# nabeelscicom/DistilCodec_nabeel

Hardware: AMD Instinct MI355X
Metric: 24 kHz samples/s encode+decode at 1/8 GPU; code-index bit-exact vs CPU (higher is better)
Workload: dtype f32

## Files before the change

### distilcodec_nabeel_amd/csrc/dcx_api.cpp

```cpp
#include "dcx_host.h"

namespace {

void prof_collect(dcx_codec* h) {
  if (h->pending.empty()) return;
  hipDeviceSynchronize();
  for (auto& r : h->pending) {
    float ms = 0.f;
    hipEventElapsedTime(&ms, h->events[r.ev0], h->events[r.ev1]);
    h->prof_launches[r.id] += 1;
    h->prof_ms[r.id] += ms;
    h->prof_flops[r.id] += r.flops;
    h->prof_bytes[r.id] += r.bytes;
  }
  h->pending.clear();
  h->ev_used = 0;
}

constexpr int kPlanMagic = 0x52414731, kPlanHead = 8;
enum { PLAN_MAGIC = 0, PLAN_BATCH, PLAN_FRAMES, PLAN_SAMPLES, PLAN_T16, PLAN_T4, PLAN_RUN, PLAN_RW };
constexpr int64_t kRaggedMaxSamples = INT32_MAX, kRaggedMaxFrames = 1 << 20, kRaggedMaxBatch = 1 << 20;
int64_t plan_words(int64_t batch) { return kPlanHead + 5 * (batch + 1); }

bool seg_from_plan(const int32_t* host, const int32_t* dev, int64_t batch, int64_t samples, int64_t frames,
// ... 473 lines not shown
  if (cin % 16 || cout % 32) return DCX_ERR_INVALID_ARG;
  if (transposed && (k % stride || (k - stride) % 2 || stride > dcx::kMaxPhases)) return DCX_ERR_INVALID_ARG;
  if (!transposed && (k % 2 == 0)) return DCX_ERR_INVALID_ARG;
  auto c = new (std::nothrow) dcx_conv();
  if (!c) return DCX_ERR_OOM;
  dcx_codec* h = &c->scratch;
  HostTensor wt;
  const int64_t n = (int64_t)cin * cout * k;
  wt.shape = transposed ? std::vector<int64_t>{cin, cout, k} : std::vector<int64_t>{cout, cin, k};
  wt.data.assign(weight, weight + n);
  h->host["c.weight"] = wt;
  HostTensor bt;
  bt.shape = {cout};
  if (bias) bt.data.assign(bias, bias + cout); else bt.data.assign(cout, 0.f);
  h->host["c.bias"] = bt;
  const int code = build_conv(h, cin, cout, k, dilation, transposed != 0, stride, c->w);
  h->host.clear();
  if (code != DCX_OK) {
    dcx_conv_destroy(c);
    return code;
  }
  *out = c;
  return DCX_OK;
}

int dcx_conv_forward(dcx_conv* c, int32_t gemm_mode, const float* x, int32_t batch, int64_t lin, float* y,
                     float* y_silu, const float* res, int32_t epi, void* stream) {
  if (!c || !x || batch <= 0 || lin <= 0 || (!y && !y_silu)) return DCX_ERR_INVALID_ARG;
  if (epi != dcx::EPI_BIAS && epi != dcx::EPI_GELU && epi != dcx::EPI_RES) return DCX_ERR_INVALID_ARG;
  if (epi == dcx::EPI_RES && !res) return DCX_ERR_INVALID_ARG;
  dcx_codec* h = &c->scratch;
  h->gemm_mode = gemm_mode;
  hipStream_t s = (hipStream_t)stream;
  CAct xa(x, nullptr);
  if (gemm_mode != DCX_GEMM_F32 && gemm_mode != DCX_GEMM_X6 && gemm_mode != DCX_GEMM_BF16) return DCX_ERR_INVALID_ARG;
  if (gemm_mode != DCX_GEMM_F32 && !f32_input_ok(c->w)) {
    const size_t need = (size_t)batch * lin * c->w.cin * 3;
    if (!grow(c->planes, c->planes_cap, need)) return DCX_ERR_OOM;
    const bool h3 = c->h3 && (c->w.taps >= 2 ? takes_h3_conv(h, c->w, lin) : takes_h3(h, c->w));
    if (h3) {
      const long long rows = (long long)batch * lin;
      const size_t words = (size_t)batch + (size_t)std::max<long long>(batch, rows);
      if (!grow(c->range, c->range_cap, words)) return DCX_ERR_OOM;
      float* am = reinterpret_cast<float*>(c->range);
      int* ash = c->range + batch;
      xa.r = Rng{};
      if (c->w.taps >= 2) {
        if (dcx::launch_h2_ranged(x, nullptr, c->planes, batch, lin, c->w.cin, 0, 0.f, am, ash, h->rflag, s) != hipSuccess)
          return fail(h, DCX_ERR_HIP, "h3 input split (per clip) failed");
        xa.r.ash = ash;
        xa.r.amax = am;
      } else {
        if (dcx::launch_h2_rows(x, c->planes, rows, c->w.cin, ash, s) != hipSuccess)
          return fail(h, DCX_ERR_HIP, "h3 input split (per row) failed: Cin must be 256, 512, 768 or 1024");
        xa.r.ash_row = ash;
      }
      xa.h2 = true;
    } else if (dcx::launch_split_planes(x, c->planes, (long long)batch * lin, c->w.cin, 0, s) != hipSuccess) {
      return DCX_ERR_HIP;
    }
    xa.p = c->planes;
  }
  ConvCall cc = framed(xa, batch, (int)lin, c->w.cin);
  cc.y = y;
  cc.y2 = y_silu;
  cc.res = res;
  cc.epi = epi;
  return run_conv(h, c->w, cc, s);
}

void dcx_conv_destroy(dcx_conv* c) {
  if (!c) return;
  if (c->planes) hipFree(c->planes);
  if (c->range) hipFree(c->range);
  for (void* p : c->scratch.allocs) hipFree(p);
  delete c;
}

const char* dcx_conv_last_kernel(const dcx_conv* c) { return c ? c->scratch.last_kname : ""; }

int dcx_conv_set_knob(dcx_conv* c, const char* name, int32_t value) {
  if (!c || !name) return DCX_ERR_INVALID_ARG;
  const auto k = knob_slot(name);
  if (!k) return fail(&c->scratch, DCX_ERR_INVALID_ARG, std::string("unknown knob: ") + name);
  c->scratch.knobs.*k = value;
  return DCX_OK;
}

int dcx_conv_set_h3(dcx_conv* c, int32_t on) {
  if (!c) return DCX_ERR_INVALID_ARG;
  c->h3 = on != 0;
  return DCX_OK;
}

int dcx_profile_enable(dcx_codec* h, int32_t on) {
  if (!h) return DCX_ERR_INVALID_ARG;
  h->prof = on != 0;
  return DCX_OK;
}

int dcx_profile_reset(dcx_codec* h) {
  if (!h) return DCX_ERR_INVALID_ARG;
  prof_collect(h);
  for (size_t i = 0; i < h->prof_names.size(); ++i) {
    h->prof_launches[i] = 0;
    h->prof_ms[i] = h->prof_flops[i] = h->prof_bytes[i] = 0;
  }
// ... 33 lines not shown
```

### distilcodec_nabeel_amd/csrc/dcx_conv_h3.hip

```cpp
#include "dcx_conv_common.h"
#include "dcx_conv_launch.h"
#include "dcx_conv_pingpong.h"

namespace dcx {

DCX_DIAG_FILE(h3)

typedef _Float16 f16x8 __attribute__((ext_vector_type(8)));

template <int BM, int BN>
__device__ __forceinline__ bool ragged_tile_done(const ConvParams& p, const ConvParams& pr, int wg, int b, int ph) {
  int q0, co0;
  tile_origin<BM, BN>(p, wg, q0, co0);
  if (!tile_dead(p, pr, b, q0)) return false;
  epilogue_dead<BM, BN, 512>(p, pr, q0, co0, b, ph);
  return true;
}

template <int BN, int HALO, bool RAG = false>
__device__ __forceinline__ void x3dq_tile(const ConvParams& p, const ConvParams& pr, const int wg, const int b, const int ph) {
  constexpr int BM = 32768 / BN, WN = BN / 64, WM = 8 / WN;
  constexpr int NA = HALO ? 2 : 3;
  constexpr int WR = BM / WM, WC = BN / WN, TM = WR / 16, TN = WC / 16;
  constexpr int AR = BM + HALO;
  constexpr int A_G = AR / 16, B_G = BN / 16;
  constexpr int A_PW = A_G / 4, B_PW = B_G / 4;
  constexpr int ABUF = AR * 128, BBUF = BN * 128;
  constexpr int LDS_B = NA * ABUF + 3 * BBUF;
  static_assert(WR == 64 && WC == 64 && A_G % 4 == 0 && B_G % 4 == 0 && AR % 64 == 0, "tile shape");
  static_assert(LDS_B <= 160 * 1024, "LDS");
  __shared__ __attribute__((aligned(16))) unsigned short lds[LDS_B / 2];

  if constexpr (RAG)
    if (ragged_tile_done<BM, BN>(p, pr, wg, b, ph)) return;
  const TileGeo g = tile_geo<BM, BN, WN>(p, wg, ph, p.Cin / 32);
  const int lane = g.lane, group = g.group, gw = g.gw, wm = g.wm, wn = g.wn, q0 = g.q0, co0 = g.co0;
  const int nchunks = g.nchunks, taps = g.taps, nsteps = g.nsteps, lo_rel = g.lo_rel, row0 = g.row0;
  const int arow = p.ldx * 4;
  const __amdgpu_buffer_rsrc_t rx = x_desc<4, HALO>(p, b, row0, BM);
  const int rbase = HALO ? row0 : 0;
  const __amdgpu_buffer_rsrc_t rw = __builtin_amdgcn_make_buffer_rsrc(
      (void*)(p.w3 + (long long)ph * taps * nchunks * p.Cout * 64), 0, taps * nchunks * p.Cout * 128, 0x00020000);

  int a_off[A_PW], b_off[B_PW];
#pragma unroll
  for (int i = 0; i < A_PW; ++i) {
    const int u = (group * A_G + i * 4 + gw) * 64;
    const int pc = u / AR, row = u - pc * AR + lane;
    a_off[i] = (rbase + row) * arow + (pc & 3) * 32 + (pc >> 2) * 16;
  }
#pragma unroll
  for (int i = 0; i < B_PW; ++i) {
    const int u = (group * B_G + i * 4 + gw) * 64;
    const int pc = u / BN, col = u - pc * BN + lane;
    b_off[i] = (co0 + col) * 128 + (pc & 3) * 32 + (pc >> 2) * 16;
  }
  unsigned short* const a_dst = lds + (group * A_G + gw) * 512;
  unsigned short* const b_dst = lds + NA * ABUF / 2 + (group * B_G + gw) * 512;
  [[maybe_unused]] bool in_loop = false;
  auto dma_step = [&](int c, int m, int slot) {
#ifdef DCX_X3_NODMA
    if (in_loop) return 0;
#endif
    int n = B_PW;
    if (m == 0) {
#pragma unroll
      for (int i = 0; i < A_PW; ++i)
        dma16(rx, a_dst + (HALO ? (c & 1) : slot) * (ABUF / 2) + i * 2048, a_off[i] + c * 128, 0);
      n += A_PW;
    }
    const int soff = (m * nchunks + c) * p.Cout * 128;
#pragma unroll
    for (int i = 0; i < B_PW; ++i) dma16(rw, b_dst + slot * (BBUF / 2) + i * 2048, b_off[i], soff);
    return n;
  };

  const int l15 = lane & 15, kg = lane >> 4;
  const int pah = kg * AR * 16, pal = (4 + kg) * AR * 16;
  const int pbh = kg * BN * 16, pbl = (4 + kg) * BN * 16;
  const char* const ldsb = reinterpret_cast<const char*>(lds);
  const int bcol = NA * ABUF + (wn * WC + l15) * 16;
  s16x8 aq[TM][2], bq[TN][2];
  auto readF = [&](int c, int m, int slot) {
    const char* a = ldsb + (HALO ? (c & 1) : slot) * ABUF + (wm * WR + m * p.in_step - lo_rel + l15) * 16;
    const char* bb = ldsb + bcol + slot * BBUF;
#pragma unroll
    for (int j = 0; j < TN; ++j) {
      bq[j][0] = *reinterpret_cast<const s16x8*>(bb + j * 256 + pbh);
      bq[j][1] = *reinterpret_cast<const s16x8*>(bb + j * 256 + pbl);
    }
#pragma unroll
    for (int i = 0; i < TM; ++i) {
      aq[i][0] = *reinterpret_cast<const s16x8*>(a + i * 256 + pah);
      aq[i][1] = *reinterpret_cast<const s16x8*>(a + i * 256 + pal);
    }
  };
  f32x4 acc[TM][TN];
  zero_acc(acc);
  auto mfma = [&]() {
    __builtin_amdgcn_s_setprio(1);
#pragma unroll
    for (int k = 0; k < 3; ++k) {
      const int sa = k == 1 ? 1 : 0, sb = k == 0 ? 1 : 0;
#pragma unroll
      for (int i = 0; i < TM; ++i)
#pragma unroll
        for (int j = 0; j < TN; ++j)
          acc[i][j] = __builtin_amdgcn_mfma_f32_16x16x32_f16(__builtin_bit_cast(f16x8, aq[i][sa]),
                                                             __builtin_bit_cast(f16x8, bq[j][sb]), acc[i][j], 0, 0, 0);
    }
    __builtin_amdgcn_s_setprio(0);
  };

  const StepPos l3 = pingpong3_prologue(nsteps, taps, dma_step);
  const EpiPre epre = epi_range_pre<HALO == 0 ? 3 : 0>(p, pr, b);
  const float unscale = __builtin_bit_cast(float, __builtin_amdgcn_readfirstlane(__builtin_bit_cast(int,
      __builtin_ldexpf(1.0f, -(p.w3_shift + (pr.x_ash ? pr.x_ash[b] : pr.x_ash_c))))));
  pingpong3_drain();
  in_loop = true;
  pingpong3_loop<true>(group, nsteps, taps, l3, dma_step, readF, mfma);
#pragma unroll
  for (int i = 0; i < TM; ++i)
#pragma unroll
    for (int j = 0; j < TN; ++j) acc[i][j] *= unscale;
// ... 1 lines not shown
}

template <int BN, int HALO, bool RAG = false>
__global__ void __launch_bounds__(512, 2) conv_gemm_x3dq(const ConvParams p) {
  int wg, b, ph;
  flat_tile(((p.Lq + 32768 / BN - 1) / (32768 / BN)) * (p.Cout / BN), p.batch, wg, b, ph);
  x3dq_tile<BN, HALO, RAG>(p, p, wg, b, ph);
}

template <int BN, bool RAG = false>
__global__ void __launch_bounds__(512, 2) conv_gemm_x3dq_group(const ConvGroup g) {
  ConvParams p;
  int local, b;
  const ConvParams& pr = group_member(g, p, local, b);
  x3dq_tile<BN, 64, RAG>(p, pr, local, b, 0);
}

template <int HALO, bool SPLIT, int BN = 256, bool RAG = false>
__device__ __forceinline__ void x3dw_tile(const ConvParams& p, const ConvParams& pr, const int wg, const int b, const int ph) {
  constexpr int BM = BN == 256 ? 256 : 384, WN = BN / 128, WM = 8 / WN;
  constexpr int WR = BM / WM, WC = 128, TM = WR / 16, TN = WC / 16;
  constexpr int AR = BM + HALO;
  constexpr int A_N = AR / 8, B_N = BN / 8;
  constexpr int A_PW = A_N / 4;
  constexpr int ABUF = AR * 128, BBUF = BN * 128;
  constexpr int NA = 2;
  constexpr int LDS_B = NA * ABUF + 2 * BBUF;
  static_assert(A_N % 4 == 0 && B_N % 4 == 0 && AR % 64 == 0, "tile shape");
  static_assert(LDS_B + 16 <= 160 * 1024, "LDS");
  __shared__ __attribute__((aligned(16))) unsigned short lds[LDS_B / 2 + 8];
  unsigned int* const rd_cnt = reinterpret_cast<unsigned int*>(lds + LDS_B / 2);

  const int tid = threadIdx.x, lane = tid & 63;
  [[maybe_unused]] const int wave = tid >> 6;
  const int group = __builtin_amdgcn_readfirstlane(tid >> 8);
  const int gw = __builtin_amdgcn_readfirstlane((tid >> 6) & 3);
  const int wm = wave / WN, wn = wave % WN;
  const int ntiles = p.Cout / BN;
  const int mt = wg / ntiles, nt = wg - mt * ntiles;
  const int q0 = mt * BM, co0 = nt * BN;
  if (RAG && tile_dead(p, pr, b, q0)) {
    epilogue_dead<BM, BN, 512>(p, pr, q0, co0, b, ph);
    return;
  }
  const int nchunks = p.Cin / 32;
  const int taps = p.taps;
  const int nsteps = nchunks * taps;
  const int lo_rel = p.in_step < 0 ? (taps - 1) * p.in_step : 0;
  const int row0 = q0 + p.in_base[ph] + lo_rel;
  const int arow = p.ldx * 4;
  const __amdgpu_buffer_rsrc_t rx = x_desc<4, HALO>(p, b, row0, BM);
  const int rbase = HALO ? row0 : 0;
  const __amdgpu_buffer_rsrc_t rw = __builtin_amdgcn_make_buffer_rsrc(
      (void*)(p.w3 + (long long)ph * taps * nchunks * p.Cout * 64), 0, taps * nchunks * p.Cout * 128, 0x00020000);

  const int a_lane = (rbase + lane) * arow;
  const int b_lane = (co0 + lane) * 128;
  [[maybe_unused]] bool in_loop = false;
  auto dmaA1 = [&](int c, int slot, int i) {
#ifdef DCX_X3_NODMA
    if (in_loop) return;
#endif
    const int k = i * 4 + gw;
    const int u = k * 64, pc = u / AR, row = u - pc * AR;
    const int abuf = HALO ? (c & 1) : slot;
    dma16(rx, lds + abuf * (ABUF / 2) + k * 512, a_lane + row * arow + (pc & 3) * 32 + (pc >> 2) * 16 + c * 128, 0);
  };
#ifndef DCX_X3W_BG0_DIV
#define DCX_X3W_BG0_DIV 2
#endif
  constexpr int B_G0 = !SPLIT ? B_N : HALO ? B_N / DCX_X3W_BG0_DIV : 0;
  constexpr int B_W0 = B_G0 / 4, B_W1 = (B_N - B_G0) / 4;
  auto dmaB1 = [&](int c, int m, int slot, int i) {
#ifdef DCX_X3_NODMA
    if (in_loop) return;
#endif
    const int k = (group ? B_G0 : 0) + i * 4 + gw;
    const int u = k * 64, pc = u / BN, col = u - pc * BN;
    dma16(rw, lds + NA * ABUF / 2 + slot * (BBUF / 2) + k * 512, b_lane + col * 128 + (pc & 3) * 32 + (pc >> 2) * 16,
          (m * nchunks + c) * p.Cout * 128);
  };
  auto dma_step = [&](int c, int m, int slot) {
    if (m == 0) {
#pragma unroll
      for (int i = 0; i < A_PW; ++i) dmaA1(c, slot, i);
    }
#pragma unroll
    for (int i = 0; i < B_W0; ++i) dmaB1(c, m, slot, i);
  };
  auto dma_step1 = [&](int c, int m, int slot) {
#pragma unroll
    for (int i = 0; i < B_W1; ++i) dmaB1(c, m, slot, i);
  };

  const int l15 = lane & 15, kg = lane >> 4;
  const char* const ldsb = reinterpret_cast<const char*>(lds);
  const char* const a_rd = ldsb + kg * AR * 16 + (wm * WR + l15) * 16;
  const char* const b_rd = ldsb + NA * ABUF + kg * BN * 16 + (wn * WC + l15) * 16;
  s16x8 aq[TM][2], bq[TN][2];
  auto readF = [&](int c, int m, int slot) {
    const char* a = a_rd + ((HALO ? (c & 1) : slot) * ABUF + (m * p.in_step - lo_rel) * 16);
    const char* bb = b_rd + slot * BBUF;
#pragma unroll
    for (int j = 0; j < TN; ++j) {
      bq[j][0] = *reinterpret_cast<const s16x8*>(bb + j * 256);
      bq[j][1] = *reinterpret_cast<const s16x8*>(bb + j * 256 + 4 * BN * 16);
    }
#pragma unroll
    for (int i = 0; i < TM; ++i) {
      aq[i][0] = *reinterpret_cast<const s16x8*>(a + i * 256);
      aq[i][1] = *reinterpret_cast<const s16x8*>(a + i * 256 + 4 * AR * 16);
    }
  };
  f32x4 acc[TM][TN];
  zero_acc(acc);
  auto mfma = [&]() {
    __builtin_amdgcn_s_setprio(1);
#pragma unroll
    for (int k = 0; k < 3; ++k) {
      const int sa = k == 1 ? 1 : 0, sb = k == 0 ? 1 : 0;
#pragma unroll
      for (int i = 0; i < TM; ++i) {
#pragma unroll
        for (int j = 0; j < TN; ++j)
          acc[i][j] = __builtin_amdgcn_mfma_f32_16x16x32_f16(__builtin_bit_cast(f16x8, aq[i][sa]),
                                                             __builtin_bit_cast(f16x8, bq[j][sb]), acc[i][j], 0, 0, 0);
      }
    }
    __builtin_amdgcn_s_setprio(0);
  };

  int cl = 0, ml = 0;
  if (SPLIT && tid == 0) *rd_cnt = 0u;
// ... 213 lines not shown
```

### distilcodec_nabeel_amd/csrc/dcx_misc.hip

```cpp
#include "dcx_kernels.h"
#include "dcx_planes.h"
#include "dcx_ln.h"

#include <algorithm>

namespace dcx {

template <int NV>
__global__ void __launch_bounds__(256) ln_rows_kernel(const float* __restrict__ x, float* __restrict__ y,
                                                       unsigned short* __restrict__ y6, int y6c, const float* __restrict__ w,
                                                       const float* __restrict__ b, long long rows, float eps, int cf,
                                                       int* ash_row, float* amax_row) {
  const int lane = threadIdx.x & 63;
  const long long row = (long long)blockIdx.x * 4 + (threadIdx.x >> 6);
  if (row >= rows) return;
  constexpr int C = 256 * NV;
  f32x4 v[NV];
#pragma unroll
  for (int i = 0; i < NV; ++i) v[i] = *reinterpret_cast<const f32x4*>(x + row * C + (lane + 64 * i) * 4);
  ln_finish<NV>(v, C, eps, cf, w, b, y ? y + row * C : nullptr, y6, y6c, row, lane, ash_row, amax_row);
}

hipError_t launch_ln_rows(const float* x, float* y, unsigned short* y6, int y6c, const float* w, const float* b,
                          long long rows, int C, float eps, int cf, hipStream_t s, int* ash_row, float* amax_row) {
// ... 288 lines not shown
    m = fmaxf(m, fmaxf(fmaxf(fabsf(v.x), fabsf(v.y)), fmaxf(fabsf(v.z), fabsf(v.w))));
  }
  range_report(m, amax, b, __builtin_inff(), nullptr, range_cur(amax, b));
}

__global__ void __launch_bounds__(256) h2_ranged_kernel(const float* __restrict__ x, float* __restrict__ yf,
                                                         unsigned short* __restrict__ y6, long long L, int C, int silu,
                                                         float floor, const float* __restrict__ amax, int* ash,
                                                         int* rflag, const int* __restrict__ clip_len, int len_mul) {
  const int b = blockIdx.y;
  const long long live4 = clip_len ? std::min<long long>(L, (long long)max(clip_len[b], 0) * len_mul) * C / 4 : L * C / 4;
  const float bound = fmaxf(amax[b], floor);
  const int sh = h2_shift(bound);
  const float sc = __builtin_ldexpf(1.0f, sh);
  if (blockIdx.x == 0 && threadIdx.x == 0) {
    ash[b] = sh;
    if (rflag && !(bound <= 3.0e38f)) atomicOr(rflag, RANGE_NONFINITE);
  }
  const long long n4 = L * C / 4, base = (long long)b * L * C;
  for (long long i4 = (long long)blockIdx.x * 256 + threadIdx.x; i4 < n4; i4 += (long long)gridDim.x * 256) {
    const long long i = base + i4 * 4;
    const f32x4 v = i4 < live4 ? *reinterpret_cast<const f32x4*>(x + i) : f32x4{0.f, 0.f, 0.f, 0.f};
    float o[4];
#pragma unroll
    for (int e = 0; e < 4; ++e) o[e] = silu ? v[e] * __builtin_amdgcn_rcpf(1.0f + __expf(-v[e])) : v[e];
    if (yf) *reinterpret_cast<f32x4*>(yf + i) = f32x4{o[0], o[1], o[2], o[3]};
    store_h2_4(y6, i / C, C, (int)(i % C), o[0], o[1], o[2], o[3], sc);
  }
}

template <int NV>
__global__ void __launch_bounds__(256) h2_rows_kernel(const float* __restrict__ x, unsigned short* __restrict__ y6,
                                                       long long rows, int* __restrict__ ash_row) {
  const int lane = threadIdx.x & 63;
  const long long row = (long long)blockIdx.x * 4 + (threadIdx.x >> 6);
  if (row >= rows) return;
  constexpr int C = 256 * NV;
  f32x4 v[NV];
  float am = 0.f;
#pragma unroll
  for (int i = 0; i < NV; ++i) {
    v[i] = *reinterpret_cast<const f32x4*>(x + row * C + (lane + 64 * i) * 4);
    am = fmaxf(am, fmaxf(fmaxf(fabsf(v[i].x), fabsf(v[i].y)), fmaxf(fabsf(v[i].z), fabsf(v[i].w))));
  }
#pragma unroll
  for (int off = 32; off >= 1; off >>= 1) am = fmaxf(am, __shfl_xor(am, off, 64));
  const int sh = h2_shift(am);
  const float sc = __builtin_ldexpf(1.0f, sh);
  if (lane == 0) ash_row[row] = sh;
#pragma unroll
  for (int i = 0; i < NV; ++i) store_h2_4(y6, row, C, (lane + 64 * i) * 4, v[i].x, v[i].y, v[i].z, v[i].w, sc);
}

hipError_t launch_h2_rows(const float* x, unsigned short* y6, long long rows, int C, int* ash_row, hipStream_t s) {
  if (!x || !y6 || !ash_row || rows < 0) return hipErrorInvalidValue;
  if (rows == 0) return hipSuccess;
  dim3 grid((unsigned)((rows + 3) / 4)), block(256);
  switch (C) {
    case 256: hipLaunchKernelGGL(h2_rows_kernel<1>, grid, block, 0, s, x, y6, rows, ash_row); break;
    case 512: hipLaunchKernelGGL(h2_rows_kernel<2>, grid, block, 0, s, x, y6, rows, ash_row); break;
    case 768: hipLaunchKernelGGL(h2_rows_kernel<3>, grid, block, 0, s, x, y6, rows, ash_row); break;
    case 1024: hipLaunchKernelGGL(h2_rows_kernel<4>, grid, block, 0, s, x, y6, rows, ash_row); break;
    default: return hipErrorInvalidValue;
  }
  return hipGetLastError();
}

__global__ void __launch_bounds__(256) zero_words_kernel(unsigned* p, long long n) {
  for (long long i = (long long)blockIdx.x * 256 + threadIdx.x; i < n; i += (long long)gridDim.x * 256) p[i] = 0u;
}

hipError_t launch_zero_words(void* p, long long n, hipStream_t s) {
  if (n <= 0) return hipSuccess;
  if (!p) return hipErrorInvalidValue;
  const long long nb = (n + 255) / 256;
  hipLaunchKernelGGL(zero_words_kernel, dim3((unsigned)std::min<long long>(nb, 1024)), dim3(256), 0, s, (unsigned*)p, n);
  return hipGetLastError();
}

hipError_t launch_clip_amax(const float* x, int batch, long long L, int C, float* amax, hipStream_t s,
                            const int* clip_len, int len_mul) {
  if (C % 4 || L < 0 || batch < 1 || batch > 65535 || !amax) return hipErrorInvalidValue;
  hipError_t e = launch_zero_words(amax, batch, s);
  if (e != hipSuccess) return e;
  const long long n4 = L * C / 4;
  const unsigned gx = (unsigned)std::max<long long>(1, std::min<long long>((n4 + 255) / 256, std::max(1, 4096 / batch)));
  if (n4 > 0) hipLaunchKernelGGL(clip_amax_kernel, dim3(gx, batch), dim3(256), 0, s, x, n4, amax, clip_len, len_mul, C / 4);
  return hipGetLastError();
}

hipError_t launch_h2_ranged(const float* x, float* yf, unsigned short* y6, int batch, long long L, int C, int silu,
                            float floor, float* amax, int* ash, int* rflag, hipStream_t s, const int* clip_len,
                            int len_mul) {
  if (C % 32 || L < 0 || batch < 1 || batch > 65535 || !y6 || !amax || !ash) return hipErrorInvalidValue;
  hipError_t e = launch_zero_words(amax, batch, s);
  if (e != hipSuccess) return e;
  const long long n4 = L * C / 4;
  const long long nb = (n4 + 255) / 256;
  const unsigned gx = (unsigned)std::max<long long>(1, std::min<long long>(nb, std::max(1, 4096 / batch)));
  if (n4 > 0) hipLaunchKernelGGL(clip_amax_kernel, dim3(gx, batch), dim3(256), 0, s, x, n4, amax, clip_len, len_mul, C / 4);
  hipLaunchKernelGGL(h2_ranged_kernel, dim3(gx, batch), dim3(256), 0, s, x, yf, y6, L, C, silu, floor, amax, ash, rflag,
                     clip_len, len_mul);
  return hipGetLastError();
}

__global__ void __launch_bounds__(256) split_planes_kernel(const float* __restrict__ x, unsigned short* __restrict__ y6,
                                                            long long rows, int C, int compact) {
  const long long total4 = rows * C / 4;
  for (long long i4 = (long long)blockIdx.x * blockDim.x + threadIdx.x; i4 < total4;
       i4 += (long long)gridDim.x * blockDim.x) {
// ... 520 lines not shown
```

### distilcodec_nabeel_amd/csrc/dcx_resblock.hip

```cpp
#include <algorithm>
#include <cstdio>

#include "dcx_resblock_common.h"

namespace dcx {

template <int C>
constexpr int kRpRows = C == 32 ? 496 : 176;
template <int C>
constexpr int kRp3Rows = C == 32 ? 624 : 240;

template <int C, bool MEAN, int RR = kRpRows<C>>
__global__ void __launch_bounds__(512, 1) conv_res_pair(const ResPairParams p) {
  using A = RpX6;
  using G = RpGeom<A, C, RR>;
  constexpr int NCH = G::NCH, WR = G::WR, RB = G::RB1, PS = G::PS, IMG = G::IMG, WTAP = G::WTAP, NIT = G::NIT;
  constexpr int TPS = C == 32 ? 2 : 1;
  constexpr int WSLOT = TPS * WTAP;
  constexpr int WP = WSLOT / 1024, WPW = (WP + 7) / 8;
  constexpr int LDS = IMG + 2 * WSLOT + G::BIASB;
  static_assert(WSLOT % 1024 == 0 && LDS <= 160 * 1024, "LDS");
  __shared__ __attribute__((aligned(16))) char lds[LDS];
  float* const bias_lds = reinterpret_cast<float*>(lds + IMG + 2 * WSLOT);

// ... 236 lines not shown
      };
      tap(acc, 8 - hk, nrb2, rp_next_tap<G>(p, m, 1, 0), res_hook);
      tap(acc, 9 - hk, nrb2, rp_next_tap<G>(p, m, 1, 1), pf_hook0);
      tap(acc, 10 - hk, nrb2, rp_next_tap<G>(p, m, 1, 2), pf_hook1);
      for (int j = 3; j < k; ++j) tap(acc, 8 + j - hk, nrb2, rp_next_tap<G>(p, m, 1, j), no_hook);
      RP_T(te);
      rp_epilogue<A, G, C, MEAN>(p, bias_lds + (kMaxGroup + m) * C, acc, res, macc, ln, m, cb0, r0, nrb2);
      RP_T(tf);
      if (has_next) {
        rp_barrier();
        rp_fill_commit<A, G>(lds, pf, nsr0, L, tid);
        rp_barrier();
      }
      RP_STAMP({
        RP_T(tg);
        st.member(ta, tb, tc, te, tf, tg, k);
      })
    }
    if (!tl.more) break;
    tl.advance();
  }
  asm volatile("s_waitcnt vmcnt(0)" ::: "memory");
  RP_STAMP(st.flush(C, tid);)
}

template <int C, bool MEAN, int RR = kRp3Rows<C>, bool RING = false, bool RAG = false>
__global__ void __launch_bounds__(512, 1) conv_res_pair_h3(const ResPairParams p) {
#ifdef __HIP_DEVICE_COMPILE__
  using A = RpH3;
  using G = RpGeom<A, C, RR>;
  constexpr int NCH = G::NCH, WR = G::WR, RB = G::RB1, PS = G::PS, IMG = G::IMG, NIT = G::NIT, WTAP = G::WTAP;
  constexpr int NSLOT = 4, RINGB = RING ? NSLOT * WTAP : 0, BIASB = G::BIASB;
  constexpr int NP = C * C / 256, PPW = (NP + 7) / 8;
  static_assert(IMG + RINGB + BIASB + 2 * NSLOT * 4 <= 160 * 1024, "LDS");
  __shared__ __attribute__((aligned(16))) char lds[IMG + RINGB + BIASB + (RING ? 2 * NSLOT * 4 : 0)];
  float* const bias_lds = reinterpret_cast<float*>(lds + IMG + RINGB);
  unsigned* const rd_cnt = reinterpret_cast<unsigned*>(lds + IMG + RINGB + BIASB);
  unsigned* const full_cnt = rd_cnt + NSLOT;

  const RpLane ln = RpLane::make<G>();
  const int tid = ln.tid, lane = ln.lane, wave = ln.wave, wc = ln.wc, wr = ln.wr;
  const int L = p.L, nmem = p.nmem;

  f32x4 pf[NIT][2];
  s16x8 wf[NCH][2][2];
  const A::Wo wo = A::wo(lane, wc);
  const A::Xb xl = A::xlane<G::NS>(lds, lane);

  int ring_t = 0;
  int ic_m = 0, ic_conv = 0, ic_j = 0;
  int dsrc[PPW];
#pragma unroll
  for (int i = 0; i < PPW; ++i) {
    const int pc = min(wave + 8 * i, NP - 1);
    const int pl = pc & 1, cbk = (pc >> 1) % (C / 16), ch = (pc >> 1) / (C / 16);
    dsrc[i] = (ch * C + cbk * 16 + ln.l15) * 128 + (lane >> 4) * 32 + pl * 16;
  }
  auto mpick = [&](auto a0, auto a1, auto a2, int m) { return m == 0 ? a0 : m == 1 ? a1 : a2; };
  auto ring_issue = [&](int slot) {
    const unsigned short* w1 = mpick(p.w1[0], p.w1[1], p.w1[2], ic_m);
    const unsigned short* w2 = mpick(p.w2[0], p.w2[1], p.w2[2], ic_m);
    const unsigned short* wp = (ic_conv ? w2 : w1) + (long long)ic_j * (WTAP / 2);
    const __amdgpu_buffer_rsrc_t rw = __builtin_amdgcn_make_buffer_rsrc((void*)wp, 0, WTAP, 0x00020000);
#pragma unroll
    for (int i = 0; i < PPW; ++i) {
      const int pc = wave + 8 * i;
      if (NP % 8 == 0 || pc < NP)
        __builtin_amdgcn_raw_ptr_buffer_load_lds(rw, (rp_lds_t)(lds + IMG + slot * WTAP + pc * 1024), 16, dsrc[i], 0, 0, 0);
    }
    if (++ic_j == mpick(p.taps[0], p.taps[1], p.taps[2], ic_m)) {
      ic_j = 0;
      if (ic_conv == 0) ic_conv = 1;
      else {
        ic_conv = 0;
        ic_m = ic_m + 1 < nmem ? ic_m + 1 : 0;
      }
    }
  };
  auto spin_ge = [&](const unsigned* c, unsigned want) {
    const unsigned a = (unsigned)(size_t)(const __attribute__((address_space(3))) void*)c;
    for (;;) {
      unsigned v;
      asm volatile("ds_read_b32 %0, %1\n\ts_waitcnt lgkmcnt(0)" : "=v"(v) : "v"(a) : "memory");
      if (__builtin_amdgcn_readfirstlane(v) >= want) break;
      __builtin_amdgcn_s_sleep(1);
    }
  };
  auto count_in = [&](unsigned* c) {
    const unsigned a = (unsigned)(size_t)(__attribute__((address_space(3))) void*)c;
    if (lane == 0) asm volatile("ds_add_u32 %0, %1" ::"v"(a), "v"(1u) : "memory");
  };
  const int wrd = lane * 16 + (2 * wc) * 2 * 1024;
  auto read_wf = [&](int slot, int ch) {
    const char* wb = lds + IMG + slot * WTAP + wrd;
#pragma unroll
    for (int cb = 0; cb < 2; ++cb) {
      wf[ch][cb][0] = *reinterpret_cast<const s16x8*>(wb + ((ch * (C / 16) + cb) * 2 + 0) * 1024);
      wf[ch][cb][1] = *reinterpret_cast<const s16x8*>(wb + ((ch * (C / 16) + cb) * 2 + 1) * 1024);
    }
  };

  auto tap = [&](RpRow (&acc)[RB], int rowoff, int nrb, const unsigned short* wnext, int nyoung, auto hook) {
    const A::Xb x = A::at(xl, (wr * 16 + rowoff) * 16);
    const int t = ring_t;
    if constexpr (RING) {
      hook();
      asm volatile("s_waitcnt lgkmcnt(0)" ::: "memory");
      count_in(rd_cnt + t % NSLOT);
      rp_wait(nyoung);
// ... 254 lines not shown
```

### distilcodec_nabeel_amd/csrc/dcx_resblock_common.h

```cpp
#pragma once
#include "dcx_kernels.h"
#include "dcx_planes.h"

namespace dcx {

typedef float f32x4 __attribute__((ext_vector_type(4)));
typedef short s16x8 __attribute__((ext_vector_type(8)));
typedef short s16x4 __attribute__((ext_vector_type(4)));
typedef __bf16 bf16x8 __attribute__((ext_vector_type(8)));
typedef _Float16 f16x8 __attribute__((ext_vector_type(8)));

__device__ __forceinline__ float rp_silu(float v) { return v * __builtin_amdgcn_rcpf(1.0f + __expf(-v)); }
__device__ __forceinline__ void rp_barrier() { asm volatile("s_waitcnt lgkmcnt(0)\n\ts_barrier" ::: "memory"); }
typedef __attribute__((address_space(3))) void* rp_lds_t;
__device__ __forceinline__ void rp_wait(int n) {
#define RP_W(k) \
  case k: asm volatile("s_waitcnt vmcnt(" #k ")" ::: "memory"); break;
  switch (n) {
    RP_W(1) RP_W(2) RP_W(3) RP_W(4) RP_W(5) RP_W(6) RP_W(7) RP_W(8) RP_W(9) RP_W(10) RP_W(11) RP_W(12)
    RP_W(13) RP_W(14) RP_W(15) RP_W(16) RP_W(17) RP_W(18) RP_W(19) RP_W(20) RP_W(21) RP_W(22) RP_W(23) RP_W(24)
    RP_W(25) RP_W(26) RP_W(27) RP_W(28) RP_W(29) RP_W(30) RP_W(31) RP_W(32)
    default: asm volatile("s_waitcnt vmcnt(0)" ::: "memory");
  }
#undef RP_W
}


struct RpX6 {
  static constexpr int PPC = 6, CW = 16, WB = 6;
  __device__ static __forceinline__ int piece(int g8) { return (g8 >> 1) * 6 + (g8 & 1) * 3; }
  __device__ static __forceinline__ float scaled(float v, float) { return v; }
  template <class T>
  __device__ static __forceinline__ T pre(T acc, float, T bias) { return acc + bias; }
  template <int N>
  __device__ static __forceinline__ void put(char* d, int ps, const float (&v)[N]) {
    typedef short vec __attribute__((ext_vector_type(N)));
    vec hv, mv, lv;
#pragma unroll
    for (int e = 0; e < N; ++e) {
      unsigned short h, m, l;
      split3(v[e], h, m, l);
      hv[e] = (short)h;
      mv[e] = (short)m;
      lv[e] = (short)l;
    }
    *reinterpret_cast<vec*>(d) = hv;
    *reinterpret_cast<vec*>(d + ps) = mv;
    *reinterpret_cast<vec*>(d + 2 * ps) = lv;
  }
  struct Wo { int o0, o1; };
  __device__ static __forceinline__ Wo wo(int lane, int wc) {
    const int l15 = lane & 15, hf = (lane >> 4) & 1, t = lane >> 5;
    const int base = ((2 * wc) * 16 + l15) * 96 + hf * 48;
    return {base + t * 16, base + (t ? 32 : 0)};
  }
  struct Xb { const char *x0, *x1, *x2; };
  template <int NS>
  __device__ static __forceinline__ Xb xlane(const char* lds, int lane) {
    const int l15 = lane & 15, hf = (lane >> 4) & 1, t = lane >> 5;
    return {lds + ((hf * 3 + t) * NS + l15) * 16, lds + ((hf * 3 + (t ? 0 : 1)) * NS + l15) * 16,
            lds + ((hf * 3 + (t ? 0 : 2)) * NS + l15) * 16};
  }
  __device__ static __forceinline__ Xb at(const Xb& x, int tb) { return {x.x0 + tb, x.x1 + tb, x.x2 + tb}; }
  struct Xv { s16x8 x2, x1, x0; };
  __device__ static __forceinline__ Xv read(const Xb& x, int io) {
    return {*reinterpret_cast<const s16x8*>(x.x2 + io), *reinterpret_cast<const s16x8*>(x.x1 + io),
            *reinterpret_cast<const s16x8*>(x.x0 + io)};
  }
  __device__ static __forceinline__ f32x4 mma(f32x4 acc, const s16x8 (&wf)[2], const Xv& v) {
    const bf16x8 w0 = __builtin_bit_cast(bf16x8, wf[0]), w1 = __builtin_bit_cast(bf16x8, wf[1]);
    acc = __builtin_amdgcn_mfma_f32_16x16x32_bf16(w1, __builtin_bit_cast(bf16x8, v.x2), acc, 0, 0, 0);
    acc = __builtin_amdgcn_mfma_f32_16x16x32_bf16(w0, __builtin_bit_cast(bf16x8, v.x1), acc, 0, 0, 0);
    return __builtin_amdgcn_mfma_f32_16x16x32_bf16(w0, __builtin_bit_cast(bf16x8, v.x0), acc, 0, 0, 0);
  }
};

struct RpH3 {
  static constexpr int PPC = 8, CW = 32, WB = 4;
  __device__ static __forceinline__ int piece(int g8) { return (g8 >> 2) * 8 + (g8 & 3); }
  __device__ static __forceinline__ float scaled(float v, float sc) { return v * sc; }
  template <class T>
  __device__ static __forceinline__ T pre(T acc, float us, T bias) { return acc * us + bias; }
  template <int N>
  __device__ static __forceinline__ void put(char* d, int ps, const float (&v)[N]) {
    typedef short vec __attribute__((ext_vector_type(N)));
    vec hv, lv;
#pragma unroll
    for (int e = 0; e < N; ++e) {
      unsigned short hh, ll;
      split2h_nc(v[e], hh, ll);
      hv[e] = (short)hh;
      lv[e] = (short)ll;
    }
    *reinterpret_cast<vec*>(d) = hv;
    *reinterpret_cast<vec*>(d + 4 * ps) = lv;
  }
  struct Wo { int o0, o1; };
  __device__ static __forceinline__ Wo wo(int lane, int wc) {
    const int base = ((2 * wc) * 16 + (lane & 15)) * 128 + (lane >> 4) * 32;
    return {base, base + 16};
  }
  struct Xb { const char *xh, *xl; };
  template <int NS>
  __device__ static __forceinline__ Xb xlane(const char* lds, int lane) {
    const int l15 = lane & 15, kg = lane >> 4;
    return {lds + (kg * NS + l15) * 16, lds + ((4 + kg) * NS + l15) * 16};
  }
  __device__ static __forceinline__ Xb at(const Xb& x, int tb) { return {x.xh + tb, x.xl + tb}; }
  struct Xv { s16x8 xl, xh; };
  __device__ static __forceinline__ Xv read(const Xb& x, int io) {
    return {*reinterpret_cast<const s16x8*>(x.xl + io), *reinterpret_cast<const s16x8*>(x.xh + io)};
  }
  __device__ static __forceinline__ f32x4 mma(f32x4 acc, const s16x8 (&wf)[2], const Xv& v) {
    const f16x8 w0 = __builtin_bit_cast(f16x8, wf[0]), w1 = __builtin_bit_cast(f16x8, wf[1]);
    acc = __builtin_amdgcn_mfma_f32_16x16x32_f16(w0, __builtin_bit_cast(f16x8, v.xl), acc, 0, 0, 0);
    acc = __builtin_amdgcn_mfma_f32_16x16x32_f16(w1, __builtin_bit_cast(f16x8, v.xh), acc, 0, 0, 0);
    return __builtin_amdgcn_mfma_f32_16x16x32_f16(w0, __builtin_bit_cast(f16x8, v.xh), acc, 0, 0, 0);
  }
};

struct RpRow {
  f32x4 c[2];
  __device__ __forceinline__ void zero() { c[0] = c[1] = f32x4{0.f, 0.f, 0.f, 0.f}; }
};

template <class A>
__device__ __forceinline__ void rp_block(RpRow& acc, const s16x8 (&wf)[2][2], const typename A::Xb& x, int io) {
  const typename A::Xv v = A::read(x, io);
#pragma unroll
  for (int cb = 0; cb < 2; ++cb) acc.c[cb] = A::mma(acc.c[cb], wf[cb], v);
}

template <class A, int C, int RR>
struct RpGeom {
  static constexpr int R = RR;
  static constexpr int M1 = R + 16;
  static constexpr int H1 = 32;
  static constexpr int NS = M1 + 2 * H1;
  static constexpr int NCH = C / A::CW;
  static constexpr int WC = C / 32, WR = 8 / WC;
  static constexpr int NB1 = M1 / 16, RB1 = NB1 / WR;
  static constexpr int NB2 = R / 16, RB2 = (NB2 + WR - 1) / WR;
  static constexpr int PS = NS * 16;
  static constexpr int IMG = NCH * A::PPC * PS;
  static constexpr int WTAP = C * C * A::WB;
  static constexpr int WROW = A::CW * A::WB;
  static constexpr int G8 = C / 8;
  static constexpr int NIT = (NS * G8 + 511) / 512;
  static constexpr int BIASB = 2 * kMaxGroup * C * 4;
  static_assert(NB1 % WR == 0 && RB1 == RB2, "row blocks per wave");
  static_assert(IMG + BIASB <= 160 * 1024, "LDS");
};

// ... 191 lines not shown
```

### distilcodec_nabeel_amd/csrc/dcx_weights.cpp

```cpp
#include "dcx_host.h"

namespace dcx::host {

struct Err {
  int code;
  std::string msg;
};

static const HostTensor* find(dcx_codec* h, const std::string& k) {
  auto it = h->host.find(k);
  return it == h->host.end() ? nullptr : &it->second;
}

static bool get_weight(dcx_codec* h, const std::string& prefix, HostTensor& out) {
  if (auto t = find(h, prefix + ".weight")) {
    out = *t;
    return true;
  }
  const char* pairs[2][2] = {{".parametrizations.weight.original0", ".parametrizations.weight.original1"},
                             {".weight_g", ".weight_v"}};
  for (auto& pr : pairs) {
    auto g = find(h, prefix + pr[0]);
    auto v = find(h, prefix + pr[1]);
    if (g && v) {
      out.shape = v->shape;
      out.data.resize(v->data.size());
      const int64_t d0 = v->shape[0], inner = v->numel() / d0;
      if ((int64_t)g->data.size() != d0) return false;
      for (int64_t i = 0; i < d0; ++i) {
        double nrm = 0;
        for (int64_t j = 0; j < inner; ++j) nrm += (double)v->data[i * inner + j] * v->data[i * inner + j];
        nrm = std::sqrt(nrm);
        const double sc = (double)g->data[i] / nrm;
        for (int64_t j = 0; j < inner; ++j) out.data[i * inner + j] = (float)(sc * v->data[i * inner + j]);
      }
      return true;
    }
  }
  return false;
}

static void split3_host(float x, unsigned short& h, unsigned short& m, unsigned short& l) {
  h = bf16_rne(x);
  const float r1 = x - bf16_f(h);
  m = bf16_rne(r1);
  const float r2 = r1 - bf16_f(m);
  l = bf16_rne(r2);
}

float round_up(double v) {
  float f = (float)v;
  if ((double)f < v) f = std::nextafter(f, INFINITY);
  return f;
// ... 5 lines not shown
  Err e{DCX_OK, ""};

  bool bad() const { return e.code != DCX_OK; }
  void set(int c, const std::string& m) {
    if (!bad()) e = {c, m};
  }

  void* upload_raw(const void* src, size_t bytes, const char* what = "weights") {
    if (bad() || dry) return nullptr;
    void* p = nullptr;
    if (hipMalloc(&p, bytes + 16) != hipSuccess) {
      set(DCX_ERR_OOM, std::string("hipMalloc failed while uploading ") + what);
      return nullptr;
    }
    h->allocs.push_back(p);
    if (hipMemcpy(p, src, bytes, hipMemcpyHostToDevice) != hipSuccess) {
      set(DCX_ERR_HIP, std::string("hipMemcpy failed while uploading ") + what);
      return nullptr;
    }
    return p;
  }
  float* upload(const std::vector<float>& v) { return (float*)upload_raw(v.data(), v.size() * sizeof(float)); }
  unsigned short* upload16(const std::vector<unsigned short>& v) {
    return (unsigned short*)upload_raw(v.data(), v.size() * sizeof(unsigned short), "split weights");
  }
  unsigned short* split_pack(const std::vector<float>& pk, int phases, int cout, int taps, int cin) {
    if (bad() || dry) return nullptr;
    const int nch = cin / 16;
    std::vector<unsigned short> out((size_t)phases * taps * nch * cout * 48);
    for (int r = 0; r < phases; ++r)
      for (int m = 0; m < taps; ++m)
        for (int c = 0; c < nch; ++c)
          for (int o = 0; o < cout; ++o) {
            unsigned short* dst = &out[((((size_t)r * taps + m) * nch + c) * cout + o) * 48];
            const float* src = &pk[(((size_t)r * cout + o) * taps + m) * cin + c * 16];
            for (int hh = 0; hh < 2; ++hh)
              for (int j = 0; j < 8; ++j) {
                unsigned short a, b2, c2;
                split3_host(src[hh * 8 + j], a, b2, c2);
                dst[hh * 24 + 0 + j] = a;
                dst[hh * 24 + 8 + j] = b2;
                dst[hh * 24 + 16 + j] = c2;
              }
          }
    return upload16(out);
  }
  unsigned short* h2_pack(const std::vector<float>& pk, int phases, int cout, int taps, int cin, int& shift) {
    if (bad() || dry) return nullptr;
    float mx = 0.f;
    for (float v : pk) mx = std::max(mx, std::fabs(v));
    int e = 0;
    if (mx > 0.f) std::frexp(mx, &e);
    shift = mx > 0.f ? 15 - e : 0;
    const int nch = cin / 32;
    std::vector<unsigned short> out((size_t)phases * taps * nch * cout * 64);
    for (int r = 0; r < phases; ++r)
    for (int m = 0; m < taps; ++m)
      for (int c = 0; c < nch; ++c)
        for (int o = 0; o < cout; ++o) {
          unsigned short* dst = &out[((((size_t)r * taps + m) * nch + c) * cout + o) * 64];
          const float* src = &pk[(((size_t)r * cout + o) * taps + m) * cin + c * 32];
          for (int j = 0; j < 32; ++j) {
            const float x = std::ldexp(src[j], shift);
            const _Float16 hh = (_Float16)x;
            const _Float16 ll = (_Float16)(x - (float)hh);
            dst[(j >> 3) * 16 + (j & 7)] = __builtin_bit_cast(unsigned short, hh);
            dst[(j >> 3) * 16 + 8 + (j & 7)] = __builtin_bit_cast(unsigned short, ll);
          }
        }
    return upload16(out);
  }
  unsigned short* compact_pack(const std::vector<float>& pk, int cout, int cin) {
    if (bad() || dry) return nullptr;
    std::vector<unsigned short> out((size_t)cout * cin);
    for (int st = 0; st < cin / 32; ++st)
      for (int o = 0; o < cout; ++o)
        for (int j = 0; j < 32; ++j) out[((size_t)st * cout + o) * 32 + j] = bf16_rne(pk[(size_t)o * cin + st * 32 + j]);
    return upload16(out);
  }
  float* alloc(size_t n) {
    if (bad() || dry) return nullptr;
    void* p = nullptr;
    if (hipMalloc(&p, n * sizeof(float) + 16) != hipSuccess) {
      set(DCX_ERR_OOM, "hipMalloc failed");
      return nullptr;
    }
    h->allocs.push_back(p);
    return (float*)p;
  }

  const HostTensor* need(const std::string& k, std::vector<int64_t> shape) {
    auto t = find(h, k);
    if (!t) {
      set(DCX_ERR_MISSING_WEIGHT, "missing checkpoint tensor '" + k + "'");
      return nullptr;
    }
    if (t->numel() != [&] { int64_t n = 1; for (auto s : shape) n *= s; return n; }()) {
      set(DCX_ERR_INVALID_ARG, "checkpoint tensor '" + k + "' has the wrong number of elements");
      return nullptr;
    }
    return t;
  }
  float* vec(const std::string& k, int64_t n) {
    auto t = need(k, {n});
    return t ? upload(t->data) : nullptr;
  }
  float* vec_bf16(const std::string& k, int64_t n) {
    auto t = need(k, {n});
    if (!t) return nullptr;
    std::vector<float> r(t->data.size());
    for (size_t i = 0; i < r.size(); ++i) r[i] = bf16_f(bf16_rne(t->data[i]));
    return upload(r);
  }
  HostTensor weight(const std::string& prefix, std::vector<int64_t> shape) {
    HostTensor w;
    if (bad()) return w;
    if (!get_weight(h, prefix, w)) {
      set(DCX_ERR_MISSING_WEIGHT, "missing checkpoint weight '" + prefix + "'");
      return w;
    }
    int64_t n = 1;
    for (auto s : shape) n *= s;
// ... 300 lines not shown
```

Baseline: 46.54 million.

## Re-layout packed h3 weights for contiguous per-lane DMA and add narrow row split

Packed hi/lo f16 weights move to a Cout-dependent layout defined in a shared header. For Cout multiples of 128, adjacent output channels become contiguous 16-byte pieces, so each lane's buffer DMA is coalesced instead of strided by 128 bytes. Resblock kernels use a 16-column pair layout. A narrow per-row h2 split kernel is added for channel counts below 256. Host packing and device offset math must stay in sync, so any mismatch would corrupt results.

```diff
diff --git a/distilcodec_nabeel_amd/csrc/dcx_api.cpp b/distilcodec_nabeel_amd/csrc/dcx_api.cpp
--- a/distilcodec_nabeel_amd/csrc/dcx_api.cpp
+++ b/distilcodec_nabeel_amd/csrc/dcx_api.cpp
@@ -549,7 +549,7 @@
         xa.r.amax = am;
       } else {
         if (dcx::launch_h2_rows(x, c->planes, rows, c->w.cin, ash, s) != hipSuccess)
-          return fail(h, DCX_ERR_HIP, "h3 input split (per row) failed: Cin must be 256, 512, 768 or 1024");
+          return fail(h, DCX_ERR_HIP, "h3 input split (per row) failed: Cin must be 256, 512, 768, 1024 or a multiple of 32 below 256");
         xa.r.ash_row = ash;
       }
       xa.h2 = true;
diff --git a/distilcodec_nabeel_amd/csrc/dcx_conv_h3.hip b/distilcodec_nabeel_amd/csrc/dcx_conv_h3.hip
--- a/distilcodec_nabeel_amd/csrc/dcx_conv_h3.hip
+++ b/distilcodec_nabeel_amd/csrc/dcx_conv_h3.hip
@@ -1,6 +1,7 @@
 #include "dcx_conv_common.h"
 #include "dcx_conv_launch.h"
 #include "dcx_conv_pingpong.h"
+#include "dcx_w3_layout.h"
 
 namespace dcx {
 
@@ -40,7 +41,7 @@
   const __amdgpu_buffer_rsrc_t rx = x_desc<4, HALO>(p, b, row0, BM);
   const int rbase = HALO ? row0 : 0;
   const __amdgpu_buffer_rsrc_t rw = __builtin_amdgcn_make_buffer_rsrc(
-      (void*)(p.w3 + (long long)ph * taps * nchunks * p.Cout * 64), 0, taps * nchunks * p.Cout * 128, 0x00020000);
+      (void*)(p.w3 + w3_step(taps, p.Cin, p.Cout, ph, 0, 0)), 0, taps * nchunks * p.Cout * 128, 0x00020000);
 
   int a_off[A_PW], b_off[B_PW];
 #pragma unroll
@@ -51,9 +52,7 @@
   }
 #pragma unroll
   for (int i = 0; i < B_PW; ++i) {
-    const int u = (group * B_G + i * 4 + gw) * 64;
-    const int pc = u / BN, col = u - pc * BN + lane;
-    b_off[i] = (co0 + col) * 128 + (pc & 3) * 32 + (pc >> 2) * 16;
+    b_off[i] = w3_wide_lane(co0, lane) + w3_wide_piece(BN, group * B_G + i * 4 + gw);
   }
   unsigned short* const a_dst = lds + (group * A_G + gw) * 512;
   unsigned short* const b_dst = lds + NA * ABUF / 2 + (group * B_G + gw) * 512;
@@ -69,7 +68,7 @@
         dma16(rx, a_dst + (HALO ? (c & 1) : slot) * (ABUF / 2) + i * 2048, a_off[i] + c * 128, 0);
       n += A_PW;
     }
-    const int soff = (m * nchunks + c) * p.Cout * 128;
+    const int soff = w3_step_bytes(nchunks, p.Cout, m, c);
 #pragma unroll
     for (int i = 0; i < B_PW; ++i) dma16(rw, b_dst + slot * (BBUF / 2) + i * 2048, b_off[i], soff);
     return n;
@@ -177,10 +176,10 @@
   const __amdgpu_buffer_rsrc_t rx = x_desc<4, HALO>(p, b, row0, BM);
   const int rbase = HALO ? row0 : 0;
   const __amdgpu_buffer_rsrc_t rw = __builtin_amdgcn_make_buffer_rsrc(
-      (void*)(p.w3 + (long long)ph * taps * nchunks * p.Cout * 64), 0, taps * nchunks * p.Cout * 128, 0x00020000);
+      (void*)(p.w3 + w3_step(taps, p.Cin, p.Cout, ph, 0, 0)), 0, taps * nchunks * p.Cout * 128, 0x00020000);
 
   const int a_lane = (rbase + lane) * arow;
-  const int b_lane = (co0 + lane) * 128;
+  const int b_lane = w3_wide_lane(co0, lane);
   [[maybe_unused]] bool in_loop = false;
   auto dmaA1 = [&](int c, int slot, int i) {
 #ifdef DCX_X3_NODMA
@@ -201,9 +200,7 @@
     if (in_loop) return;
 #endif
     const int k = (group ? B_G0 : 0) + i * 4 + gw;
-    const int u = k * 64, pc = u / BN, col = u - pc * BN;
-    dma16(rw, lds + NA * ABUF / 2 + slot * (BBUF / 2) + k * 512, b_lane + col * 128 + (pc & 3) * 32 + (pc >> 2) * 16,
-          (m * nchunks + c) * p.Cout * 128);
+    dma16(rw, lds + NA * ABUF / 2 + slot * (BBUF / 2) + k * 512, b_lane, w3_step_bytes(nchunks, p.Cout, m, c) + w3_wide_piece(BN, k));
   };
   auto dma_step = [&](int c, int m, int slot) {
     if (m == 0) {
diff --git a/distilcodec_nabeel_amd/csrc/dcx_misc.hip b/distilcodec_nabeel_amd/csrc/dcx_misc.hip
--- a/distilcodec_nabeel_amd/csrc/dcx_misc.hip
+++ b/distilcodec_nabeel_amd/csrc/dcx_misc.hip
@@ -364,10 +364,30 @@
   for (int i = 0; i < NV; ++i) store_h2_4(y6, row, C, (lane + 64 * i) * 4, v[i].x, v[i].y, v[i].z, v[i].w, sc);
 }
 
+__global__ void __launch_bounds__(256) h2_rows_narrow_kernel(const float* __restrict__ x, unsigned short* __restrict__ y6,
+                                                              long long rows, int C, int* __restrict__ ash_row) {
+  const int lane = threadIdx.x & 63;
+  const long long row = (long long)blockIdx.x * 4 + (threadIdx.x >> 6);
+  if (row >= rows) return;
+  const bool on = lane * 4 < C;
+  f32x4 v = {0.f, 0.f, 0.f, 0.f};
+  if (on) v = *reinterpret_cast<const f32x4*>(x + row * C + lane * 4);
+  float am = fmaxf(fmaxf(fabsf(v.x), fabsf(v.y)), fmaxf(fabsf(v.z), fabsf(v.w)));
+#pragma unroll
+  for (int off = 32; off >= 1; off >>= 1) am = fmaxf(am, __shfl_xor(am, off, 64));
+  const int sh = h2_shift(am);
+  if (lane == 0) ash_row[row] = sh;
+  if (on) store_h2_4(y6, row, C, lane * 4, v.x, v.y, v.z, v.w, __builtin_ldexpf(1.0f, sh));
+}
+
 hipError_t launch_h2_rows(const float* x, unsigned short* y6, long long rows, int C, int* ash_row, hipStream_t s) {
   if (!x || !y6 || !ash_row || rows < 0) return hipErrorInvalidValue;
   if (rows == 0) return hipSuccess;
   dim3 grid((unsigned)((rows + 3) / 4)), block(256);
+  if (C > 0 && C < 256 && C % 32 == 0) {
+    hipLaunchKernelGGL(h2_rows_narrow_kernel, grid, block, 0, s, x, y6, rows, C, ash_row);
+    return hipGetLastError();
+  }
   switch (C) {
     case 256: hipLaunchKernelGGL(h2_rows_kernel<1>, grid, block, 0, s, x, y6, rows, ash_row); break;
     case 512: hipLaunchKernelGGL(h2_rows_kernel<2>, grid, block, 0, s, x, y6, rows, ash_row); break;
diff --git a/distilcodec_nabeel_amd/csrc/dcx_resblock.hip b/distilcodec_nabeel_amd/csrc/dcx_resblock.hip
--- a/distilcodec_nabeel_amd/csrc/dcx_resblock.hip
+++ b/distilcodec_nabeel_amd/csrc/dcx_resblock.hip
@@ -312,9 +312,7 @@
   int dsrc[PPW];
 #pragma unroll
   for (int i = 0; i < PPW; ++i) {
-    const int pc = min(wave + 8 * i, NP - 1);
-    const int pl = pc & 1, cbk = (pc >> 1) % (C / 16), ch = (pc >> 1) / (C / 16);
-    dsrc[i] = (ch * C + cbk * 16 + ln.l15) * 128 + (lane >> 4) * 32 + pl * 16;
+    dsrc[i] = w3_pair_piece(C, min(wave + 8 * i, NP - 1), lane);
   }
   auto mpick = [&](auto a0, auto a1, auto a2, int m) { return m == 0 ? a0 : m == 1 ? a1 : a2; };
   auto ring_issue = [&](int slot) {
diff --git a/distilcodec_nabeel_amd/csrc/dcx_resblock_common.h b/distilcodec_nabeel_amd/csrc/dcx_resblock_common.h
--- a/distilcodec_nabeel_amd/csrc/dcx_resblock_common.h
+++ b/distilcodec_nabeel_amd/csrc/dcx_resblock_common.h
@@ -1,6 +1,7 @@
 #pragma once
 #include "dcx_kernels.h"
 #include "dcx_planes.h"
+#include "dcx_w3_layout.h"
 
 namespace dcx {
 
@@ -97,8 +98,7 @@
   }
   struct Wo { int o0, o1; };
   __device__ static __forceinline__ Wo wo(int lane, int wc) {
-    const int base = ((2 * wc) * 16 + (lane & 15)) * 128 + (lane >> 4) * 32;
-    return {base, base + 16};
+    return {w3_pair_lane(2 * wc * 16, lane, 0), w3_pair_lane(2 * wc * 16, lane, 1)};
   }
   struct Xb { const char *xh, *xl; };
   template <int NS>
diff --git a/distilcodec_nabeel_amd/csrc/dcx_w3_layout.h b/distilcodec_nabeel_amd/csrc/dcx_w3_layout.h
--- /dev/null
+++ b/distilcodec_nabeel_amd/csrc/dcx_w3_layout.h
@@ -0,0 +1,45 @@
+#pragma once
+
+#if defined(__HIPCC__) || defined(__CUDACC__)
+#define DCX_W3_HD __host__ __device__
+#else
+#define DCX_W3_HD
+#endif
+
+namespace dcx {
+
+enum W3Flavour { kW3Cols = 0, kW3Wide = 1, kW3Pair = 2 };
+
+DCX_W3_HD constexpr W3Flavour w3_flavour(int cout) {
+  return cout % 128 == 0 ? kW3Wide : cout % 16 == 0 ? kW3Pair : kW3Cols;
+}
+
+DCX_W3_HD constexpr int w3_in_step(W3Flavour f, int co, int kg, int pl) {
+  return f == kW3Wide   ? (co >> 6) * 4096 + (pl * 4 + kg) * 512 + (co & 63) * 8
+         : f == kW3Pair ? (co >> 4) * 1024 + pl * 512 + kg * 128 + (co & 15) * 8
+                        : co * 64 + kg * 16 + pl * 8;
+}
+DCX_W3_HD constexpr long long w3_step(int taps, int cin, int cout, int r, int m, int c) {
+  return (((long long)r * taps + m) * (cin / 32) + c) * cout * 64;
+}
+DCX_W3_HD constexpr long long w3_offset(int taps, int cin, int cout, int r, int m, int ci, int co, int pl) {
+  return w3_step(taps, cin, cout, r, m, ci >> 5) + w3_in_step(w3_flavour(cout), co, (ci >> 3) & 3, pl) + (ci & 7);
+}
+
+
+DCX_W3_HD constexpr int w3_step_bytes(int nchunks, int cout, int m, int c) { return (m * nchunks + c) * cout * 128; }
+DCX_W3_HD constexpr int w3_wide_lane(int co0, int lane) { return w3_in_step(kW3Wide, co0 + lane, 0, 0) * 2; }
+DCX_W3_HD constexpr int w3_wide_piece(int bn, int k) {
+  const int u = k * 64, pc = u / bn, col = u - pc * bn;
+  return w3_in_step(kW3Wide, col, pc & 3, pc >> 2) * 2;
+}
+
+DCX_W3_HD constexpr int w3_pair_lane(int col0, int lane, int pl) {
+  return w3_in_step(kW3Pair, col0 + (lane & 15), lane >> 4, pl) * 2;
+}
+DCX_W3_HD constexpr int w3_pair_piece(int C, int pc, int lane) {
+  const int cbk = (pc >> 1) % (C / 16), ch = (pc >> 1) / (C / 16);
+  return ch * C * 128 + w3_pair_lane(cbk * 16, lane, pc & 1);
+}
+
+}
diff --git a/distilcodec_nabeel_amd/csrc/dcx_weights.cpp b/distilcodec_nabeel_amd/csrc/dcx_weights.cpp
--- a/distilcodec_nabeel_amd/csrc/dcx_weights.cpp
+++ b/distilcodec_nabeel_amd/csrc/dcx_weights.cpp
@@ -1,4 +1,5 @@
 #include "dcx_host.h"
+#include "dcx_w3_layout.h"
 
 namespace dcx::host {
 
@@ -110,22 +111,19 @@
     int e = 0;
     if (mx > 0.f) std::frexp(mx, &e);
     shift = mx > 0.f ? 15 - e : 0;
-    const int nch = cin / 32;
-    std::vector<unsigned short> out((size_t)phases * taps * nch * cout * 64);
+    std::vector<unsigned short> out((size_t)phases * taps * cin * cout * 2);
     for (int r = 0; r < phases; ++r)
     for (int m = 0; m < taps; ++m)
-      for (int c = 0; c < nch; ++c)
-        for (int o = 0; o < cout; ++o) {
-          unsigned short* dst = &out[((((size_t)r * taps + m) * nch + c) * cout + o) * 64];
-          const float* src = &pk[(((size_t)r * cout + o) * taps + m) * cin + c * 32];
-          for (int j = 0; j < 32; ++j) {
-            const float x = std::ldexp(src[j], shift);
-            const _Float16 hh = (_Float16)x;
-            const _Float16 ll = (_Float16)(x - (float)hh);
-            dst[(j >> 3) * 16 + (j & 7)] = __builtin_bit_cast(unsigned short, hh);
-            dst[(j >> 3) * 16 + 8 + (j & 7)] = __builtin_bit_cast(unsigned short, ll);
-          }
+      for (int o = 0; o < cout; ++o) {
+        const float* src = &pk[(((size_t)r * cout + o) * taps + m) * cin];
+        for (int j = 0; j < cin; ++j) {
+          const float x = std::ldexp(src[j], shift);
+          const _Float16 hh = (_Float16)x;
+          const _Float16 ll = (_Float16)(x - (float)hh);
+          out[(size_t)w3_offset(taps, cin, cout, r, m, j, o, 0)] = __builtin_bit_cast(unsigned short, hh);
+          out[(size_t)w3_offset(taps, cin, cout, r, m, j, o, 1)] = __builtin_bit_cast(unsigned short, ll);
         }
+      }
     return upload16(out);
   }
   unsigned short* compact_pack(const std::vector<float>& pk, int cout, int cin) {
```

Result: faster. 48.51 million, median of 6 (+4.2%).
